# zkonduit/ezkl

Hardware: AMD Instinct MI355X
Metric: BN254 G1 MSM pts/s (2^20 points per GPU; NTT 2^22 elems/s in extra) (higher is better)
Workload: dtype u32x8 (254-bit modular integer, Montgomery); 1 GPU; configs[1]: standalone 2^20-point BN254 G1 MSM (uniform scalars, try-and-increment bases) + 2^22 scalar-field NTT per GPU; parallelism=points sharded across 1 rank(s); all_gather of 64-B partials + host fold

## Files before the change

ezkl_amd/csrc/field.hpp:

```cpp
#pragma once
#ifndef __HIPCC_RTC__
#include <stdint.h>
#include <hip/hip_runtime.h>
#else
typedef unsigned int uint32_t;
typedef unsigned long long uint64_t;
typedef unsigned long size_t;
#endif
#include "bn254_constants.h"

#define EZ_HD __host__ __device__ __forceinline__
#define EZ_D __device__ __forceinline__

namespace ezkl {

struct alignas(16) fe_t {
    uint32_t v[8];
};
#define EZKL_FE_DEFINED 1

struct FqP {
    static constexpr uint32_t MOD[8] = BN32_FQ_MOD_INIT;
    static constexpr uint32_t ONE[8] = BN32_FQ_R_INIT;
    static constexpr uint32_t R2[8] = BN32_FQ_R2_INIT;
// ... 134 lines not shown
    EZ_HD static fe_t sub_lazy(const fe_t& a, const fe_t& b) {
        fe_t d;
        uint32_t br = 0;
#pragma unroll
        for (int i = 0; i < 8; i++) d.v[i] = subb32(a.v[i], b.v[i], br);
        uint32_t c = 0;
        fe_t r;
#pragma unroll
        for (int i = 0; i < 8; i++) r.v[i] = addc32(d.v[i], mod2(i), c);
        return r;
    }
    __host__ __device__ __attribute__((noinline)) static u32x8 mul_lazy_call(u32x8 a, u32x8 b) {
        fe_t x, y;
#pragma unroll
        for (int i = 0; i < 8; i++) { x.v[i] = a[i]; y.v[i] = b[i]; }
#if defined(__HIP_DEVICE_COMPILE__)
        fe_t r;
        mont_mul_single<P>(x.v, y.v, r.v);
#else
        fe_t r = mul_portable(reduce_once(reduce_2p(x)), y);
#endif
        u32x8 o;
#pragma unroll
        for (int i = 0; i < 8; i++) o[i] = r.v[i];
        return o;
    }
    EZ_HD static fe_t mul_lazy(const fe_t& a, const fe_t& b) {
        u32x8 x, y;
#pragma unroll
        for (int i = 0; i < 8; i++) { x[i] = a.v[i]; y[i] = b.v[i]; }
        u32x8 o = mul_lazy_call(x, y);
        fe_t r;
#pragma unroll
        for (int i = 0; i < 8; i++) r.v[i] = o[i];
        return r;
    }
    EZ_HD static fe_t mul(const fe_t& a, const fe_t& b) {
        u32x8 x, y;
#pragma unroll
        for (int i = 0; i < 8; i++) { x[i] = a.v[i]; y[i] = b.v[i]; }
        u32x8 o = mul_call(x, y);
        fe_t r;
#pragma unroll
        for (int i = 0; i < 8; i++) r.v[i] = o[i];
        return r;
    }
    EZ_HD static fe_t mul_inl(const fe_t& a, const fe_t& b) {
#if defined(__HIP_DEVICE_COMPILE__)
        return mont_mul_asm<P>(a, b);
#else
        return mul_portable(a, b);
#endif
    }
    EZ_HD static fe_t mul_portable(const fe_t& a, const fe_t& b) {
        uint32_t t[8];
#pragma unroll
        for (int i = 0; i < 8; i++) t[i] = 0;
#pragma unroll
        for (int i = 0; i < 8; i++) {
            const uint32_t bi = b.v[i];
            uint64_t A = mad_wide(a.v[0], bi, t[0]);
            const uint32_t m = (uint32_t)A * P::INV;
            uint64_t C = mad_wide(m, P::MOD[0], (uint32_t)A);
#pragma unroll
            for (int j = 1; j < 8; j++) {
                A = mad_wide(a.v[j], bi, (uint64_t)t[j] + (A >> 32));
                C = mad_wide(m, P::MOD[j], (uint64_t)(uint32_t)A + (C >> 32));
                t[j - 1] = (uint32_t)C;
            }
            t[7] = (uint32_t)(A >> 32) + (uint32_t)(C >> 32);
        }
        fe_t r;
#pragma unroll
        for (int i = 0; i < 8; i++) r.v[i] = t[i];
        return reduce_once(r);
    }
    EZ_HD static fe_t sqr(const fe_t& a) { return mul(a, a); }

    EZ_HD static fe_t from_mont(const fe_t& a) {
        fe_t o = zero();
        o.v[0] = 1;
        return mul(a, o);
    }
    EZ_HD static fe_t to_mont(const fe_t& a) { return mul(a, r2()); }

    EZ_HD static fe_t pow(const fe_t& a, const uint32_t e[8]) {
        fe_t acc = one(), base = a;
        for (int i = 0; i < 256; i++) {
            if ((e[i >> 5] >> (i & 31)) & 1) acc = mul(acc, base);
            base = sqr(base);
        }
        return acc;
    }
    EZ_HD static fe_t pow_u64(const fe_t& a, uint64_t e) {
        fe_t acc = one(), base = a;
        while (e) {
            if (e & 1) acc = mul(acc, base);
            base = sqr(base);
            e >>= 1;
        }
        return acc;
    }
    EZ_HD static fe_t inv(const fe_t& a) {
        uint32_t e[8];
        uint64_t br = 2;
        for (int i = 0; i < 8; i++) {
            uint64_t t = (uint64_t)P::MOD[i] - br;
            e[i] = (uint32_t)t;
            br = (t >> 63) & 1;
        }
        return pow(a, e);
    }
    EZ_HD static fe_t from_u64(uint64_t x) {
        fe_t t = zero();
        t.v[0] = (uint32_t)x;
        t.v[1] = (uint32_t)(x >> 32);
        return to_mont(t);
    }
};

}
namespace ezkl {
#include "montmul_gen.hpp"
template <> __device__ __forceinline__ void mont_mul_single<FqP>(const uint32_t (&a)[8], const uint32_t (&b)[8], uint32_t (&r)[8]) { mont_mul_asm1_fq(a, b, r); }
template <> __device__ __forceinline__ void mont_mul_single<FrP>(const uint32_t (&a)[8], const uint32_t (&b)[8], uint32_t (&r)[8]) { mont_mul_asm1_fr(a, b, r); }
using Fr = Field<FrP>;
using Fq = Field<FqP>;

EZ_D fe_t ld_fe(const fe_t* p) {
    const uint4* q = reinterpret_cast<const uint4*>(p);
    uint4 lo = q[0], hi = q[1];
    fe_t r;
    r.v[0] = lo.x; r.v[1] = lo.y; r.v[2] = lo.z; r.v[3] = lo.w;
    r.v[4] = hi.x; r.v[5] = hi.y; r.v[6] = hi.z; r.v[7] = hi.w;
    return r;
}
EZ_D void st_fe(fe_t* p, const fe_t& a) {
    uint4* q = reinterpret_cast<uint4*>(p);
    q[0] = make_uint4(a.v[0], a.v[1], a.v[2], a.v[3]);
    q[1] = make_uint4(a.v[4], a.v[5], a.v[6], a.v[7]);
}

EZ_HD fe_t fr_const(const uint32_t (&c)[8]) {
    fe_t r;
#pragma unroll
    for (int i = 0; i < 8; i++) r.v[i] = c[i];
    return r;
}
struct FrConst {
    static constexpr uint32_t ROOT[8] = BN32_FR_ROOT_INIT;
    static constexpr uint32_t ZETA[8] = BN32_FR_ZETA_INIT;
    static constexpr uint32_t ZETA2[8] = BN32_FR_ZETA2_INIT;
    static constexpr uint32_t DELTA[8] = BN32_FR_DELTA_INIT;
};
struct FqConst {
    static constexpr uint32_t B3[8] = BN32_FQ_B3_INIT;
};

}
```

ezkl_amd/csrc/msm.hip:

```cpp
#include "common.hpp"
#include <deque>
#include <thread>
#include <chrono>
#include "curve.hpp"
#include "curve29.hpp"
#include "host64.hpp"
#include <string.h>

namespace ezkl {

static constexpr uint32_t MSM_MAX_PART_BITS = 12;
static constexpr uint32_t MSM_SPAN_HEAVY = 16;
static constexpr uint32_t MSM_PART_STAGE = 13312;
static constexpr uint32_t MSM_BINSORT_STAGE = 15360;
static constexpr uint32_t MSM_HEAVY_CHUNK = 256;
static constexpr uint32_t MSM_DIGIT_E = 8;
static constexpr uint32_t MSM_LMIN = 8;
static constexpr uint32_t MSM_MAX_BIG = 64;
static constexpr uint32_t MSM_BIG_BLOCKS = 64;
static constexpr uint32_t MSM_BIG_ROWS = 8;

__device__ __forceinline__ uint32_t msm_part_of(uint32_t bucket, uint32_t NP) { return bucket ? 1u + (bucket & (NP - 1u)) : 0u; }
__device__ __forceinline__ uint32_t msm_lane_len(const uint32_t* offsets, uint32_t nb, uint32_t nlanes, uint32_t lmin) {
    const uint32_t l = (uint32_t)(((uint64_t)offsets[nb] + nlanes - 1) / nlanes);
// ... 54 lines not shown
    return v;
}
static const int MSM_SLOTS = msm_slots_init();
struct MsmSlot {
    hipStream_t st = nullptr;
    uint8_t* scratch = nullptr;
    size_t scratch_bytes = 0;
    uint32_t* pinned = nullptr;
    void* pinned_dev = nullptr;
    size_t pinned_msms = 0;
    hipEvent_t done = nullptr;
    uint32_t bits = 0;
    uint32_t count = 0;
    void* out = nullptr;
    bool busy = false;
};
static constexpr int MSM_CALL_SLOTS = 4;
struct MsmState {
    std::map<const Bases*, MsmTable> tables;
    hipStream_t table_stream = nullptr;
    MsmSlot slots[MSM_MAX_SLOTS];
    MsmSlot call_slots[MSM_CALL_SLOTS];
    bool call_claimed[MSM_CALL_SLOTS] = {false, false, false, false};
    bool call_finishing[MSM_CALL_SLOTS] = {false, false, false, false};
    std::thread::id call_owner[MSM_CALL_SLOTS];
    hipEvent_t call_order_ev = nullptr;
    hipStream_t copy_st = nullptr;
    fe_t* tail_pinned = nullptr;
    size_t tail_pinned_elems = 0;
    MsmUpload* open_upload = nullptr;
    MsmBatch* open_batch = nullptr;
    bool attrs_set = false;
    int acc_blocks_per_cu = 0;
};
static MsmState& msm_state() {
    Ctx* c = ctx();
    if (!c->msm_state) c->msm_state = new MsmState();
    return *static_cast<MsmState*>(c->msm_state);
}


static WinPlan pick_plan(size_t n) {
    WinPlan best{0, 0, 0};
    double best_cost = 0;
    for (uint32_t W = 10; W <= 127; W++) {
        WinPlan p{W, 254 / W, 254 % W};
        if (p.cmax() > 23) continue;
        const double cost = (double)n * W + 4.0 * (double)((size_t)1 << (p.cmax() - 1));
        if (!best.W || cost < best_cost) { best = p; best_cost = cost; }
    }
    return best;
}

__global__ __launch_bounds__(256) void msm_precompute_kernel(const g1a_t* prev, g1a_t* next, size_t n, uint32_t c) {
    size_t i = (size_t)blockIdx.x * blockDim.x + threadIdx.x;
    if (i >= n) return;
    g1a_t p = ld_g1a(prev + i);
    g1x_t a = g1x_from_affine(p);
    for (uint32_t k = 0; k < c; k++) a = g1x_double(a);
    st_g1a(next + i, g1x_to_affine(a));
}

__global__ __launch_bounds__(256) void msm_table_to_r261_kernel(g1a_t* tab, size_t count) {
    size_t i = (size_t)blockIdx.x * blockDim.x + threadIdx.x;
    if (i >= count) return;
    fe_t k;
#pragma unroll
    for (int q = 0; q < 8; q++) k.v[q] = Fq29C::R261_32[q];
    g1a_t p = ld_g1a(tab + i);
    if (g1a_is_id(p)) return;
    p.x = Fq::mul(p.x, k);
    p.y = Fq::mul(p.y, k);
    st_g1a(tab + i, p);
}

__device__ __forceinline__ bool gt_half_r(const fe_t& s) {
    uint32_t d[8], c = 0, br = 0;
#pragma unroll
    for (int i = 0; i < 8; i++) d[i] = addc32(s.v[i], s.v[i], c);
#pragma unroll
    for (int i = 0; i < 8; i++) (void)subb32(d[i], FrP::MOD[i], br);
    return c != 0 || br == 0;
}
__device__ __forceinline__ fe_t msm_canon(const fe_t* scalars, size_t i, uint32_t& neg) {
    fe_t s = Fr::from_mont(ld_fe(scalars + i));
    neg = 0;
    if (gt_half_r(s)) {
        uint32_t br = 0;
#pragma unroll
        for (int k = 0; k < 8; k++) s.v[k] = subb32(FrP::MOD[k], s.v[k], br);
        neg = 1;
    }
    return s;
}
__device__ __forceinline__ uint32_t msm_take_bits(fe_t& s, uint32_t c) {
    const uint32_t d = s.v[0] & ((1u << c) - 1u);
#pragma unroll
    for (int k = 0; k < 7; k++) s.v[k] = __builtin_amdgcn_alignbit(s.v[k + 1], s.v[k], c);
    s.v[7] >>= c;
    return d;
}
template <class F>
__device__ __forceinline__ void msm_foreach_digit(fe_t s, uint32_t neg, const WinPlan& wp, F&& f) {
    uint32_t carry = 0;
    for (uint32_t w = 0; w < wp.W; w++) {
        const uint32_t c = wp.width(w), half = 1u << (c - 1);
        uint32_t raw = msm_take_bits(s, c) + carry;
        if (raw > half) {
            carry = 1;
            if (raw != (1u << c)) f(w, (1u << c) - raw - 1u, neg ^ 1u);
        } else {
            carry = 0;
            if (raw) f(w, raw - 1u, neg);
        }
    }
}

__device__ __forceinline__ bool msm_digit_step(fe_t& s, uint32_t neg, uint32_t c, uint32_t& carry, uint32_t& bucket, uint32_t& sign) {
    const uint32_t half = 1u << (c - 1);
    const uint32_t raw = msm_take_bits(s, c) + carry;
    if (raw > half) {
        carry = 1;
        bucket = (1u << c) - raw - 1u;
        sign = neg ^ 1u;
        return raw != (1u << c);
    }
    carry = 0;
    bucket = raw - 1u;
    sign = neg;
    return raw != 0;
}

__device__ __forceinline__ uint32_t msm_block_scan(uint32_t v, uint32_t* wsum, uint32_t& total) {
    const uint32_t lane = threadIdx.x & 63u, wave = threadIdx.x >> 6, nw = blockDim.x >> 6;
    uint32_t x = v;
#pragma unroll
    for (uint32_t d = 1; d < 64; d <<= 1) {
        const uint32_t y = __shfl_up(x, d, 64);
        if (lane >= d) x += y;
    }
    if (lane == 63) wsum[wave] = x;
    __syncthreads();
    if (wave == 0) {
        uint32_t s = lane < nw ? wsum[lane] : 0u;
#pragma unroll
        for (uint32_t d = 1; d < 16; d <<= 1) {
            const uint32_t y = __shfl_up(s, d, 64);
            if (lane >= d) s += y;
        }
        if (lane < nw) wsum[lane] = s;
    }
    __syncthreads();
    total = wsum[nw - 1];
    const uint32_t r = x + (wave ? wsum[wave - 1] : 0u);
    __syncthreads();
    return r;
}

__global__ __launch_bounds__(256) void msm_hist_kernel(MsmCols cols, size_t n, size_t per_block, WinPlan wp,
                                                       uint32_t LB, uint32_t NP, uint32_t* wg_hist, uint32_t* wg_cnt,
                                                       uint32_t* zero_base, uint32_t zero_words, size_t bstride) {
    BOFF(); BSH(wg_hist); BSH(wg_cnt);
    const fe_t* scalars = msm_col(cols);
    if (zero_base) {
        BSH(zero_base);
        for (uint32_t i = blockIdx.x * 256 + threadIdx.x; i < zero_words; i += gridDim.x * 256) zero_base[i] = 0;
    }
    __shared__ uint32_t lh[(1u << MSM_MAX_PART_BITS) + 1];
    const uint32_t NQ = NP + 1;
    for (uint32_t p = threadIdx.x; p < NQ; p += 256) lh[p] = 0;
    __syncthreads();
    size_t lo = (size_t)blockIdx.x * per_block, hi = lo + per_block < n ? lo + per_block : n;
    for (size_t i0 = lo + threadIdx.x; i0 < hi; i0 += 4 * 256) {
        fe_t s[4];
        uint32_t neg[4], carry[4] = {0, 0, 0, 0};
#pragma unroll
        for (int q = 0; q < 4; q++) {
            const size_t i = i0 + (size_t)q * 256;
            if (i < hi) s[q] = msm_canon(scalars, i, neg[q]);
            else { s[q] = Fr::zero(); neg[q] = 0; }
        }
        for (uint32_t w = 0; w < wp.W; w++) {
            const uint32_t c = wp.width(w);
#pragma unroll
            for (int q = 0; q < 4; q++) {
                uint32_t bucket, sign;
                if (msm_digit_step(s[q], neg[q], c, carry[q], bucket, sign)) atomicAdd(&lh[msm_part_of(bucket, NP)], 1u);
            }
        }
    }
    __syncthreads();
    for (uint32_t p = threadIdx.x; p < NQ; p += 256) {
        wg_hist[(size_t)blockIdx.x * NQ + p] = lh[p];
        wg_cnt[(size_t)blockIdx.x * NQ + p] = lh[p];
    }
}
__global__ __launch_bounds__(1024) void msm_hist_scan_kernel(uint32_t* wg_hist, uint32_t G, uint32_t NP, uint32_t* part_count, size_t bstride) {
    BOFF(); BSH(wg_hist); BSH(part_count);
    __shared__ uint32_t sums[32][33];
    const uint32_t c = threadIdx.x & 31, j = threadIdx.x >> 5;
    const uint32_t p = blockIdx.x * 32 + c;
    const uint32_t chunk = (G + 31) / 32, g0 = j * chunk, g1 = g0 + chunk < G ? g0 + chunk : G;
    uint32_t s = 0;
    if (p < NP)
        for (uint32_t g = g0; g < g1; g++) s += wg_hist[(size_t)g * NP + p];
    sums[j][c] = s;
    __syncthreads();
    if (j == 0) {
        uint32_t run = 0;
        for (uint32_t q = 0; q < 32; q++) {
            uint32_t v = sums[q][c];
            sums[q][c] = run;
            run += v;
        }
        if (p < NP) part_count[p] = run;
    }
    __syncthreads();
    if (p < NP) {
        uint32_t run = sums[j][c];
        for (uint32_t g = g0; g < g1; g++) {
            uint32_t v = wg_hist[(size_t)g * NP + p];
            wg_hist[(size_t)g * NP + p] = run;
            run += v;
        }
    }
}
__device__ __forceinline__ void msm_part_scan_body(const uint32_t* part_count, uint32_t NQ, uint32_t* part_base, uint32_t* big_flag,
                                                   uint32_t* big_list, uint32_t* big_count, uint32_t* sh) {
    const uint32_t t = threadIdx.x;
    constexpr uint32_t PER = 5;
    uint32_t v[PER], sum = 0;
#pragma unroll
    for (uint32_t q = 0; q < PER; q++) {
        const uint32_t i = PER * t + q;
        v[q] = i < NQ ? part_count[i] : 0;
        sum += v[q];
    }
    uint32_t total;
    uint32_t run = msm_block_scan(sum, sh, total) - sum;
#pragma unroll
    for (uint32_t q = 0; q < PER; q++) {
        const uint32_t i = PER * t + q;
        if (i < NQ) part_base[i] = run;
        run += v[q];
    }
    if (t == 1023) part_base[NQ] = total;
#pragma unroll
    for (uint32_t q = 0; q < PER; q++) {
        const uint32_t i = PER * t + q;
        if (i == 0 || i >= NQ) continue;
        uint32_t slot = 0;
        if (v[q] > MSM_BINSORT_STAGE) {
            slot = atomicAdd(big_count, 1u);
            if (slot < MSM_MAX_BIG) big_list[slot] = i - 1;
            slot = slot < MSM_MAX_BIG ? slot + 1 : 0;
        }
        big_flag[i - 1] = slot;
    }
}
__global__ __launch_bounds__(1024) void msm_part_scan_kernel(const uint32_t* part_count, uint32_t NQ, uint32_t* part_base, uint32_t* big_flag,
                                                             uint32_t* big_list, uint32_t* big_count, size_t bstride) {
    BOFF(); BSH(part_count); BSH(part_base); BSH(big_flag); BSH(big_list); BSH(big_count);
    __shared__ uint32_t sh[1024];
    msm_part_scan_body(part_count, NQ, part_base, big_flag, big_list, big_count, sh);
}
__global__ __launch_bounds__(1024) void msm_partition_kernel(MsmCols cols, size_t n, size_t per_block, WinPlan wp,
                                                             uint32_t LB, uint32_t NP, size_t base_offset, size_t tab_stride,
                                                             const uint32_t* part_base, const uint32_t* wg_hist, const uint32_t* wg_cnt, uint2* entries,
                                                             uint32_t* vals, size_t bstride) {
    BOFF(); BSH(part_base); BSH(wg_hist); BSH(wg_cnt); BSH(entries); BSH(vals);
    const fe_t* scalars = msm_col(cols);
    extern __shared__ uint32_t plds[];
    __shared__ uint32_t tsum[1024];
    const uint32_t NQ = NP + 1;
    uint32_t* start = plds;
    uint32_t* cursor = plds + (NQ + 1);
    uint32_t* gbase = plds + 2 * (NQ + 1);
    uint2* stage = reinterpret_cast<uint2*>(plds + 3 * (NQ + 1));
    const uint32_t t = threadIdx.x, T = blockDim.x;
    const uint32_t K = (NQ + T - 1) / T;
    uint32_t loc = 0;
    for (uint32_t q = 0; q < K; q++) {
        const uint32_t p = t * K + q;
        if (p < NQ) loc += wg_cnt[(size_t)blockIdx.x * NQ + p];
    }
    uint32_t total;
    uint32_t run = msm_block_scan(loc, tsum, total) - loc;
    for (uint32_t q = 0; q < K; q++) {
        const uint32_t p = t * K + q;
        if (p < NQ) {
            start[p] = run;
            cursor[p] = run;
            gbase[p] = part_base[p] + wg_hist[(size_t)blockIdx.x * NQ + p];
            run += wg_cnt[(size_t)blockIdx.x * NQ + p];
        }
    }
    __syncthreads();
    const size_t lo = (size_t)blockIdx.x * per_block, hi = lo + per_block < n ? lo + per_block : n;
    const size_t i = lo + t;
    if (i < hi) {
        uint32_t neg;
        fe_t s = msm_canon(scalars, i, neg);
        msm_foreach_digit(s, neg, wp, [&](uint32_t w, uint32_t bucket, uint32_t sign) {
            const uint32_t r = atomicAdd(&cursor[msm_part_of(bucket, NP)], 1u);
            stage[r] = make_uint2((uint32_t)(w * tab_stride + base_offset + i) | (sign << 31), bucket);
        });
    }
    __syncthreads();
    const uint32_t PB = 31 - __clz(NP);
    for (uint32_t idx = t; idx < total; idx += T) {
        const uint2 e = stage[idx];
        const uint32_t p = msm_part_of(e.y, NP);
        const uint32_t slot = gbase[p] + (idx - start[p]);
        if (p) entries[slot] = make_uint2(e.x, e.y >> PB);
        else vals[slot] = e.x;
    }
}
__device__ __forceinline__ uint32_t msm_wave_rank(uint32_t* cnt, uint32_t key) {
    const uint64_t active = __ballot(1);
    const uint32_t first = __builtin_amdgcn_readfirstlane(key);
    if (__ballot(key == first) == active) {
        const uint32_t rank = (uint32_t)__popcll(active & ((1ull << (threadIdx.x & 63u)) - 1ull));
        uint32_t base = 0;
        if (rank == 0) base = atomicAdd(&cnt[first], (uint32_t)__popcll(active));
        return (uint32_t)__builtin_amdgcn_readfirstlane(base) + rank;
    }
    return atomicAdd(&cnt[key], 1u);
}
__device__ __forceinline__ void msm_bins_scan(uint32_t* cnt, uint32_t* tsum, uint32_t nbins, uint32_t p, uint32_t beg, const uint32_t* part_base,
                                              bool emit, uint32_t* offsets, g1x29_t* buckets) {
    const uint32_t t = threadIdx.x;
    uint32_t loc[4], s = 0;
#pragma unroll
    for (int q = 0; q < 4; q++) {
        uint32_t j = t * 4 + q;
        loc[q] = j < nbins ? cnt[j] : 0;
        s += loc[q];
    }
    uint32_t total;
    uint32_t run = msm_block_scan(s, tsum, total) - s;
#pragma unroll
    for (int q = 0; q < 4; q++) {
        uint32_t j = t * 4 + q;
        if (j < nbins) {
            cnt[j] = run;
            if (emit) {
                const bool b0 = (p == 0 && j == 0);
                offsets[(size_t)p * nbins + j] = b0 ? part_base[0] : beg + run;
                if (b0 ? part_base[1] == part_base[0] : loc[q] == 0) st_f29(&buckets[(size_t)p * nbins + j].zz, Fq29::zero());
            }
        }
        run += loc[q];
    }
    __syncthreads();
}
__device__ __forceinline__ void msm_bigsort_count_body(const uint2* entries, const uint32_t* part_base, uint32_t LB, const uint32_t* big_list,
                                                       const uint32_t* big_count, uint32_t* bin_total, uint32_t* block_off, uint32_t* cnt, uint32_t bx,
                                                       uint32_t by, uint32_t rows);
__global__ __launch_bounds__(512) void msm_binsort_kernel(const uint2* entries, const uint32_t* part_base, uint32_t LB, uint32_t NP,
                                                          const uint32_t* big_flag, uint32_t* offsets, uint32_t* vals, g1x29_t* buckets,
                                                          const uint32_t* big_list, const uint32_t* big_count, uint32_t* bin_total, uint32_t* block_off,
                                                          size_t bstride) {
    BOFF(); BSH(entries); BSH(part_base); BSH(big_flag); BSH(offsets); BSH(vals); BSH(buckets);
    __shared__ uint32_t cnt[2048];
    __shared__ uint32_t tsum[512];
    extern __shared__ uint32_t stage[];
    if (blockIdx.x >= NP) {
        BSH(big_list); BSH(big_count); BSH(bin_total); BSH(block_off);
        const uint32_t w = blockIdx.x - NP;
        msm_bigsort_count_body(entries, part_base, LB, big_list, big_count, bin_total, block_off, cnt, w % MSM_BIG_BLOCKS, w / MSM_BIG_BLOCKS, MSM_BIG_ROWS);
        return;
    }
    const uint32_t p = blockIdx.x, t = threadIdx.x, nbins = 1u << LB;
    const uint32_t beg = part_base[p + 1], end = part_base[p + 2];
    if (p == NP - 1 && t == 0) offsets[(size_t)NP * nbins] = end;
    if (big_flag[p]) return;
    const bool staged = (end - beg) <= MSM_BINSORT_STAGE;
    for (uint32_t j = t; j < nbins; j += 512) cnt[j] = 0;
    __syncthreads();
    if (staged) {
        constexpr int PER = MSM_BINSORT_STAGE / 512;
        uint2 v[PER];
#pragma unroll
        for (int q = 0; q < PER; q++) {
            const uint32_t e = beg + t + (uint32_t)q * 512u;
            v[q] = e < end ? entries[e] : make_uint2(0u, 0xffffffffu);
        }
#pragma unroll
        for (int q = 0; q < PER; q++)
            if (v[q].y != 0xffffffffu) atomicAdd(&cnt[v[q].y], 1u);
        __syncthreads();
        msm_bins_scan(cnt, tsum, nbins, p, beg, part_base, true, offsets, buckets);
#pragma unroll
        for (int q = 0; q < PER; q++)
            if (v[q].y != 0xffffffffu) stage[atomicAdd(&cnt[v[q].y], 1u)] = v[q].x;
        __syncthreads();
        for (uint32_t i = t; i < end - beg; i += 512) vals[beg + i] = stage[i];
    } else {
// ... 382 lines not shown
static size_t msm_group_size(const MsmTable* T, size_t n, bool small_scalars, size_t batch = 0) {
    if (const char* e = getenv("EZKL_MSM_GROUP")) {
        const int v = atoi(e);
        if (v >= 1 && v <= (int)MSM_MAX_GROUP) return (size_t)v;
    }
    (void)T; (void)n; (void)batch;
    if (small_scalars) {
        static const int small = [] { const char* e = getenv("EZKL_MSM_GROUP_SMALL"); const int v = e ? atoi(e) : 0; return v >= 1 && v <= (int)MSM_MAX_GROUP ? v : 6; }();
        return (size_t)small;
    }
    static const int big = [] { const char* e = getenv("EZKL_MSM_GROUP_BIG"); const int v = e ? atoi(e) : 0; return v >= 1 && v <= (int)MSM_MAX_GROUP ? v : 4; }();
    return (size_t)big;
}
static int msm_enqueue(Ctx* c, MsmSlot& sl, hipStream_t st, MsmTable* T, size_t base_offset, const fe_t* const* cols, size_t count, size_t n, bool timed) {
    int rc = EZKL_OK;
    if (count < 1 || count > MSM_MAX_GROUP) return EZKL_ERR_INVALID;
    const unsigned Z = (unsigned)count;
    const WinPlan wp = T->wp;
    const uint32_t W = wp.W, bits = wp.cmax() - 1;
    const uint32_t nb = 1u << bits;
    const size_t npairs = n * W;
    uint32_t PB = bits < 10 ? bits : 10;
    while (PB < bits && PB < MSM_MAX_PART_BITS && (npairs >> PB) > (size_t)MSM_BINSORT_STAGE * 9 / 10) PB++;
    const uint32_t LB = bits - PB, NP = 1u << PB;
    int& acc_blocks_per_cu = msm_state().acc_blocks_per_cu;
    if (!acc_blocks_per_cu) {
        EZ_HIP(hipFuncSetAttribute((const void*)msm_binsort_kernel, hipFuncAttributeMaxDynamicSharedMemorySize, 96 * 1024));
        EZ_HIP(hipFuncSetAttribute((const void*)msm_partition_kernel, hipFuncAttributeMaxDynamicSharedMemorySize, 144 * 1024));
        EZ_HIP(hipOccupancyMaxActiveBlocksPerMultiprocessor(&acc_blocks_per_cu, msm_accumulate_kernel, 256, 0));
        if (acc_blocks_per_cu < 1) acc_blocks_per_cu = 1;
    }
    const size_t resident = (size_t)acc_blocks_per_cu * 256 * c->num_cus;
    const size_t load = npairs >> bits, per_lane = load * 9 / 10 > 40 ? load * 9 / 10 : 40;
    size_t rounds = npairs / (resident * per_lane);
    if (rounds < 1) rounds = 1;
    uint32_t L = (uint32_t)((npairs + resident * rounds - 1) / (resident * rounds));
    if (L < 8) L = 8;
    if (const char* e = getenv("EZKL_MSM_L")) {
        const int v = atoi(e);
        if (v > 0 && v < (1 << 20)) L = (uint32_t)v;
    }
    const uint32_t nlanes = cdiv(npairs, L);
    static const uint32_t lmin = [] { const char* e = getenv("EZKL_MSM_LMIN"); const int v = e ? atoi(e) : 0; return (uint32_t)(v >= 1 && v <= 4096 ? v : (int)MSM_LMIN); }();
    constexpr uint32_t coop = 7;
    static const uint32_t span_heavy = [] { const char* e = getenv("EZKL_MSM_SPAN"); const int v = e ? atoi(e) : 0; return (uint32_t)(v >= 1 && v <= 4096 ? v : (int)MSM_SPAN_HEAVY); }();
    ReduceGeom rg;
    memset(&rg, 0, sizeof rg);
    if (LB > 0) {
        rg.wA = LB; rg.wsA = PB;
        rg.wB = (PB + 1) / 2; rg.wsB = 0;
        rg.wC = PB - rg.wB; rg.wsC = rg.wB;
    } else {
        rg.wA = (bits + 2) / 3; rg.wsA = 0;
        rg.wB = (bits - rg.wA + 1) / 2; rg.wsB = rg.wA;
        rg.wC = bits - rg.wA - rg.wB; rg.wsC = rg.wA + rg.wB;
    }
    {
        const uint32_t rows = 1u << (rg.wB + rg.wC), cols = 1u << rg.wA;
        uint32_t E = MSM_DIGIT_E;
        if (const char* e = getenv("EZKL_MSM_E")) {
            const int v = atoi(e);
            if (v > 0 && v <= 1024 && (v & (v - 1)) == 0) E = (uint32_t)v;
        }
        rg.EA = rows < E ? rows : E; rg.GA = rows / rg.EA;
        rg.ET = cols < E ? cols : E; rg.GT = cols / rg.ET;
    }
    const uint32_t nA = 1u << rg.wA, nT = 1u << (rg.wB + rg.wC);
    const uint32_t n_partA = nA * rg.GA, n_partT = nT * rg.GT;
    const uint32_t nplanes = 1 + bits;
    size_t per_block = MSM_PART_STAGE / W / 64 * 64;
    {
        const size_t lds_words = (144u << 10) / 4, fixed = 3 * ((size_t)NP + 2);
        const size_t fit = lds_words > fixed ? (lds_words - fixed) / (2 * (size_t)W) / 64 * 64 : 64;
        if (per_block > fit) per_block = fit;
    }
    if (per_block > 1024) per_block = 1024;
    if (per_block < 64) per_block = 64;
    const unsigned sgrid = cdiv(n, per_block);
    auto al = [](size_t x) { return (x + 255) & ~(size_t)255; };
    size_t off = 0;
    auto carve = [&](size_t bytes) { size_t o = off; off += al(bytes); return o; };
    size_t o_ent = carve(npairs * 8), o_vals = carve(npairs * 4), o_offs = carve(((size_t)nb + 1) * 4);
    const uint32_t NQ = NP + 1;
    size_t o_pcnt = carve((NQ + 1) * 4), o_pbase = carve((NQ + 1) * 4), o_wgh = carve((size_t)sgrid * NQ * 4), o_wgc = carve((size_t)sgrid * NQ * 4);
    size_t o_heavy = carve((size_t)nb * 4), o_chunks = carve(((size_t)nlanes + 1) * 4);
    const size_t nbins = (size_t)1 << LB;
    size_t o_hcnt = carve(256), o_btot = carve(MSM_MAX_BIG * nbins * 4), o_planes = carve((size_t)nplanes * sizeof(g1x29_t));
    const size_t zero_bytes = off - o_hcnt;
    size_t o_bflag = carve((size_t)NP * 4), o_blist = carve(MSM_MAX_BIG * 4),
           o_boff = carve((size_t)MSM_MAX_BIG * MSM_BIG_BLOCKS * nbins * 4);
    size_t o_lfirst = carve((size_t)nlanes * 4);
    size_t o_bkt = carve((size_t)nb * sizeof(g1x29_t));
    size_t o_head = carve((size_t)nlanes * sizeof(g1x29_t)), o_tail = carve((size_t)nlanes * sizeof(g1x29_t));
    size_t o_partA = carve((size_t)n_partA * sizeof(g1x29_t)), o_partT = carve((size_t)n_partT * sizeof(g1x29_t));
    size_t o_SA = carve((size_t)nA * sizeof(g1x29_t)), o_T = carve((size_t)nT * sizeof(g1x29_t));
    const size_t bstride = count > 1 ? off : 0;
    rc = slot_prepare(sl, off * count, count);
    if (rc) return rc;
    uint8_t* S = sl.scratch;
    MsmCols kcols;
    for (size_t j = 0; j < MSM_MAX_GROUP; j++) kcols.col[j] = cols[j < count ? j : 0];
    uint2* entries = (uint2*)(S + o_ent);
    uint32_t* vals = (uint32_t*)(S + o_vals);
    uint32_t* offs = (uint32_t*)(S + o_offs);
    uint32_t *pcnt = (uint32_t*)(S + o_pcnt), *pbase = (uint32_t*)(S + o_pbase), *wghist = (uint32_t*)(S + o_wgh), *wgcnt = (uint32_t*)(S + o_wgc);
    uint32_t *heavy = (uint32_t*)(S + o_heavy), *hcnt = (uint32_t*)(S + o_hcnt), *chunks = (uint32_t*)(S + o_chunks);
    uint32_t* lfirst = (uint32_t*)(S + o_lfirst);
    uint32_t *bflag = (uint32_t*)(S + o_bflag), *blist = (uint32_t*)(S + o_blist), *btot = (uint32_t*)(S + o_btot), *boff = (uint32_t*)(S + o_boff);
    uint32_t* bcnt = hcnt + 2;
    g1x29_t *bkt = (g1x29_t*)(S + o_bkt), *head = (g1x29_t*)(S + o_head), *tail = (g1x29_t*)(S + o_tail);
    g1x29_t *partA = (g1x29_t*)(S + o_partA), *partT = (g1x29_t*)(S + o_partT), *SA = (g1x29_t*)(S + o_SA), *TT = (g1x29_t*)(S + o_T);
    g1x29_t* planes = (g1x29_t*)(S + o_planes);

    hipEvent_t m0 = nullptr, m1 = nullptr, a0 = nullptr, a1 = nullptr;
    bool timed_chain = timed;
    if (timed) {
        const char* tm = getenv("EZKL_HIP_TIMING");
        if (tm && !strcmp(tm, "none")) timed = timed_chain = false;
        else if (tm && !strcmp(tm, "kernel")) timed_chain = false;
    }
    if (timed) {
        if (timed_chain && (rc = ev_pair(c, "msm", &m0, &m1))) return rc;
        if ((rc = ev_pair(c, "msm_accumulate", &a0, &a1))) return rc;
        if (timed_chain) EZ_HIP(hipEventRecord(m0, st));
    }
    hipLaunchKernelGGL(msm_hist_kernel, dim3(sgrid, 1, Z), dim3(256), 0, st, kcols, n, per_block, wp, LB, NP, wghist, wgcnt, hcnt,
                       (uint32_t)(zero_bytes / 4), bstride);
    hipLaunchKernelGGL(msm_hist_scan_kernel, dim3(cdiv(NQ, 32), 1, Z), dim3(1024), 0, st, wghist, sgrid, NQ, pcnt, bstride);
    hipLaunchKernelGGL(msm_part_scan_kernel, dim3(1, 1, Z), dim3(1024), 0, st, pcnt, NQ, pbase, bflag, blist, bcnt, bstride);
    hipLaunchKernelGGL(msm_partition_kernel, dim3(sgrid, 1, Z), dim3((unsigned)per_block), (3 * ((size_t)NQ + 1) + 2 * per_block * W) * 4, st, kcols, n, per_block, wp,
                       LB, NP, base_offset, T->n, pbase, wghist, wgcnt, entries, vals, bstride);
    hipLaunchKernelGGL(msm_binsort_kernel, dim3(NP + MSM_BIG_BLOCKS * MSM_BIG_ROWS, 1, Z), dim3(512), MSM_BINSORT_STAGE * 4, st, entries, pbase, LB, NP, bflag, offs,
                       vals, bkt, blist, bcnt, btot, boff, bstride);
    hipLaunchKernelGGL(msm_bigsort_scatter_kernel, dim3(MSM_BIG_BLOCKS, MSM_BIG_ROWS, Z), dim3(512), 0, st, entries, pbase, LB, blist, bcnt, btot, boff, offs,
                       vals, bkt, bstride);
    if (timed) EZ_HIP(hipEventRecord(a0, st));
    hipLaunchKernelGGL(msm_accumulate_kernel, dim3(cdiv(nlanes, 256), 1, Z), dim3(256), 0, st, T->tab, offs, vals, nb, nlanes, bkt, head, tail,
                       lfirst, lmin, bstride);
    if (timed) EZ_HIP(hipEventRecord(a1, st));
    if (nlanes > 1)
    {
        hipLaunchKernelGGL(msm_fixup_boundary_tree_kernel, dim3(cdiv(nlanes - 1, 256), 1, Z), dim3(256), 0, st, offs, nb, nlanes, lfirst, head, tail, bkt,
                           heavy, hcnt, chunks, lmin, span_heavy, bstride);
    }
    {
        size_t max_heavy = nlanes / span_heavy + 1;
        const size_t heavy_wgs = (max_heavy + 3) / 4;
        unsigned hb = (unsigned)(heavy_wgs < (size_t)c->num_cus * 4 ? heavy_wgs : (size_t)c->num_cus * 4);
        size_t max_chunks = nlanes / MSM_HEAVY_CHUNK + max_heavy;
        const size_t chunk_wgs = (max_chunks + 3) / 4;
        unsigned cb = (unsigned)(chunk_wgs < (size_t)c->num_cus * 4 ? chunk_wgs : (size_t)c->num_cus * 4);
        hipLaunchKernelGGL(msm_fixup_heavy1_kernel, dim3(cb, 1, Z), dim3(256), 0, st, offs, nb, nlanes, lfirst, head, tail, bkt, chunks, hcnt, lmin, coop & 4u, bstride);
        hipLaunchKernelGGL(msm_fixup_heavy2_kernel, dim3(hb, 1, Z), dim3(256), 0, st, offs, nb, nlanes, head, tail, heavy, hcnt, bkt, lmin, coop & 4u, bstride);
    }
    {
        const uint32_t th = n_partA > n_partT ? n_partA : n_partT;
        hipLaunchKernelGGL(msm_reduce1_kernel, dim3(cdiv(th, 256), 2, Z), dim3(256), 0, st, bkt, rg, partA, partT, bstride);
        auto pow2_le = [](uint32_t x) { uint32_t p = 1; while (p * 2 <= x) p *= 2; return p; };
        uint32_t lanesA = pow2_le(rg.GA < 64 ? rg.GA : 64), lanesT = pow2_le(rg.GT < 64 ? rg.GT : 64);
        auto waves = [&](uint32_t nout, uint32_t lanes) { return cdiv(nout, 64 / lanes); };
        while (waves(nA, lanesA) + waves(nT, lanesT) > (unsigned)c->num_cus * 4 && (lanesA > 1 || lanesT > 1)) {
            if (lanesT > 1 && waves(nT, lanesT) >= waves(nA, lanesA)) lanesT >>= 1; else if (lanesA > 1) lanesA >>= 1; else lanesT >>= 1;
        }
        const uint32_t blocksA = waves(nA, lanesA);
        hipLaunchKernelGGL(msm_reduce2_kernel, dim3(blocksA + waves(nT, lanesT), 1, Z), dim3(64), 0, st, partA, partT, rg, SA, TT, lanesA, lanesT, blocksA, coop & 1u, bstride);
        hipLaunchKernelGGL(msm_planes_kernel, dim3(nplanes, 1, Z), dim3(256), 0, st, SA, TT, rg, planes, (g1x29_t*)sl.pinned_dev,
                           coop & 10u, bstride);
    }
    EZ_HIP(hipGetLastError());
    if (getenv("EZKL_MSM_DEBUG")) {
        uint32_t hc = 0;
        EZ_HIP(hipMemcpyAsync(&hc, hcnt, 4, hipMemcpyDeviceToHost, st));
        EZ_HIP(hipStreamSynchronize(st));
        fprintf(stderr, "[msm] n=%zu W=%u bits=%u L=%u nlanes=%u heavy=%u\n", n, W, bits, L, nlanes, hc);
    }
    if (timed_chain) EZ_HIP(hipEventRecord(m1, st));
    EZ_HIP(hipEventRecord(sl.done, st));
    sl.bits = bits;
    sl.count = (uint32_t)count;
    sl.busy = true;
    return EZKL_OK;
}
static int msm_run_groups(Ctx* c, MsmTable* T, size_t base_offset, const fe_t* const* cols, size_t batch, size_t n, void* out_host,
                          const hipEvent_t* wait_ev, bool small_scalars) {
    const size_t G = msm_group_size(T, n, small_scalars, batch);
    static const bool dbg = getenv("EZKL_MSM_DEBUG") != nullptr;
    if (dbg) fprintf(stderr, "[ezkl_hip] msm batch: %zu columns of %zu points, %s scalars, groups of %zu\n", batch, n, small_scalars ? "witness-shaped" : "general", G);
    int rc = EZKL_OK;
    size_t gi = 0;
    for (size_t j0 = 0; j0 < batch && !rc; gi++) {
        size_t cnt = batch - j0 < G ? batch - j0 : G;
        if (wait_ev && j0 > 0) {
            const size_t left = batch - j0;
            cnt = left <= 2 ? 1 : std::min(G, (left + 1) / 2);
        }
        MsmSlot& sl = g_slots[gi % MSM_SLOTS];
        if (sl.busy) rc = msm_finish(sl);
        if (!rc) rc = slot_prepare(sl, 0);
        for (size_t j = 0; wait_ev && j < cnt && !rc; j++)
            if (hipStreamWaitEvent(sl.st, wait_ev[j0 + j], 0) != hipSuccess) rc = EZKL_ERR_HIP;
        if (!rc) {
            sl.out = (uint8_t*)out_host + 64 * j0;
            rc = msm_enqueue(c, sl, sl.st, T, base_offset, cols + j0, cnt, n, false);
        }
        j0 += cnt;
    }
    for (size_t k = 0; k < (size_t)MSM_SLOTS; k++) {
        MsmSlot& sl = g_slots[(gi + k) % MSM_SLOTS];
        if (!sl.busy) continue;
        if (!rc) rc = msm_finish(sl);
        else { (void)hipStreamSynchronize(sl.st); sl.busy = false; }
    }
    return rc;
}
// ... 464 lines not shown
```

Baseline: 811.4 million pts/s.

## Rework MSM scalar recoding, histogram scan and persistent partition kernel

Replaces from_mont (a full Montgomery multiply by one) with a dedicated REDC, and replaces the per-window shifting of all eight limbs with a streaming 64-bit buffer recoder that extracts signed digits for several scalars at once. The duplicated per-workgroup count array is dropped: the partition kernel now recovers per-tile counts by differencing adjacent exclusive-scan rows, with the partition totals serving as the last row. The histogram scan is rebuilt as a narrow-column wave-shuffle scan with XCD-aware strip mapping. The partition kernel is made persistent, with a grid capped at the CU count, and prefetches the next tile's scalars and histogram rows. The aim is to cut scalar-decoding ALU work and memory traffic in the sort front-end, at the cost of more complex indexing and less parallelism in the partition launch.

After: 822.1 million pts/s (median of 6 runs). 1.3% higher.

```diff
diff --git a/ezkl_amd/csrc/field.hpp b/ezkl_amd/csrc/field.hpp
--- a/ezkl_amd/csrc/field.hpp
+++ b/ezkl_amd/csrc/field.hpp
@@ -240,6 +240,26 @@
         o.v[0] = 1;
         return mul(a, o);
     }
+    EZ_HD static fe_t redc(const fe_t& a) {
+        uint32_t t[8];
+#pragma unroll
+        for (int i = 0; i < 8; i++) t[i] = a.v[i];
+#pragma unroll
+        for (int i = 0; i < 8; i++) {
+            const uint32_t m = t[0] * P::INV;
+            uint64_t pr[8];
+#pragma unroll
+            for (int j = 0; j < 8; j++) pr[j] = mad_wide(m, P::MOD[j], t[j]);
+            uint32_t c = 0;
+#pragma unroll
+            for (int j = 0; j < 7; j++) t[j] = addc32((uint32_t)pr[j + 1], (uint32_t)(pr[j] >> 32), c);
+            t[7] = (uint32_t)(pr[7] >> 32) + c;
+        }
+        fe_t r;
+#pragma unroll
+        for (int i = 0; i < 8; i++) r.v[i] = t[i];
+        return reduce_once(r);
+    }
     EZ_HD static fe_t to_mont(const fe_t& a) { return mul(a, r2()); }
 
     EZ_HD static fe_t pow(const fe_t& a, const uint32_t e[8]) {
diff --git a/ezkl_amd/csrc/msm.hip b/ezkl_amd/csrc/msm.hip
--- a/ezkl_amd/csrc/msm.hip
+++ b/ezkl_amd/csrc/msm.hip
@@ -160,8 +160,8 @@
     for (int i = 0; i < 8; i++) (void)subb32(d[i], FrP::MOD[i], br);
     return c != 0 || br == 0;
 }
-__device__ __forceinline__ fe_t msm_canon(const fe_t* scalars, size_t i, uint32_t& neg) {
-    fe_t s = Fr::from_mont(ld_fe(scalars + i));
+__device__ __forceinline__ fe_t msm_canon(const fe_t& mont, uint32_t& neg) {
+    fe_t s = Fr::redc(mont);
     neg = 0;
     if (gt_half_r(s)) {
         uint32_t br = 0;
@@ -171,42 +171,34 @@
     }
     return s;
 }
-__device__ __forceinline__ uint32_t msm_take_bits(fe_t& s, uint32_t c) {
-    const uint32_t d = s.v[0] & ((1u << c) - 1u);
-#pragma unroll
-    for (int k = 0; k < 7; k++) s.v[k] = __builtin_amdgcn_alignbit(s.v[k + 1], s.v[k], c);
-    s.v[7] >>= c;
-    return d;
-}
-template <class F>
-__device__ __forceinline__ void msm_foreach_digit(fe_t s, uint32_t neg, const WinPlan& wp, F&& f) {
-    uint32_t carry = 0;
-    for (uint32_t w = 0; w < wp.W; w++) {
-        const uint32_t c = wp.width(w), half = 1u << (c - 1);
-        uint32_t raw = msm_take_bits(s, c) + carry;
-        if (raw > half) {
-            carry = 1;
-            if (raw != (1u << c)) f(w, (1u << c) - raw - 1u, neg ^ 1u);
-        } else {
-            carry = 0;
-            if (raw) f(w, raw - 1u, neg);
-        }
-    }
-}
-
-__device__ __forceinline__ bool msm_digit_step(fe_t& s, uint32_t neg, uint32_t c, uint32_t& carry, uint32_t& bucket, uint32_t& sign) {
-    const uint32_t half = 1u << (c - 1);
-    const uint32_t raw = msm_take_bits(s, c) + carry;
-    if (raw > half) {
-        carry = 1;
-        bucket = (1u << c) - raw - 1u;
-        sign = neg ^ 1u;
-        return raw != (1u << c);
-    }
-    carry = 0;
-    bucket = raw - 1u;
-    sign = neg;
-    return raw != 0;
+template <int Q, class F>
+__device__ __forceinline__ void msm_recode(const fe_t (&s)[Q], const uint32_t (&neg)[Q], const WinPlan& wp, F&& f) {
+    uint64_t buf[Q];
+    uint32_t carry[Q];
+#pragma unroll
+    for (int q = 0; q < Q; q++) { buf[q] = 0; carry[q] = 0; }
+    uint32_t have = 0, w = 0, c = wp.width(0);
+#pragma unroll
+    for (int k = 0; k < 8; k++) {
+#pragma unroll
+        for (int q = 0; q < Q; q++) buf[q] |= (uint64_t)s[q].v[k] << have;
+        have += 32;
+        while (have >= c && w < wp.W) {
+            const uint32_t full = 1u << c, half = full >> 1;
+#pragma unroll
+            for (int q = 0; q < Q; q++) {
+                const uint32_t raw = ((uint32_t)buf[q] & (full - 1u)) + carry[q];
+                buf[q] >>= c;
+                const uint32_t minus = raw > half ? 1u : 0u;
+                const uint32_t mag = minus ? full - raw : raw;
+                carry[q] = minus;
+                if (mag) f(q, w, mag - 1u, neg[q] ^ minus);
+            }
+            have -= c;
+            w++;
+            c = wp.width(w);
+        }
+    }
 }
 
 __device__ __forceinline__ uint32_t msm_block_scan(uint32_t v, uint32_t* wsum, uint32_t& total) {
@@ -236,9 +228,9 @@
 }
 
 __global__ __launch_bounds__(256) void msm_hist_kernel(MsmCols cols, size_t n, size_t per_block, WinPlan wp,
-                                                       uint32_t LB, uint32_t NP, uint32_t* wg_hist, uint32_t* wg_cnt,
+                                                       uint32_t LB, uint32_t NP, uint32_t* wg_hist,
                                                        uint32_t* zero_base, uint32_t zero_words, size_t bstride) {
-    BOFF(); BSH(wg_hist); BSH(wg_cnt);
+    BOFF(); BSH(wg_hist);
     const fe_t* scalars = msm_col(cols);
     if (zero_base) {
         BSH(zero_base);
@@ -251,56 +243,77 @@
     size_t lo = (size_t)blockIdx.x * per_block, hi = lo + per_block < n ? lo + per_block : n;
     for (size_t i0 = lo + threadIdx.x; i0 < hi; i0 += 4 * 256) {
         fe_t s[4];
-        uint32_t neg[4], carry[4] = {0, 0, 0, 0};
+        uint32_t neg[4];
 #pragma unroll
         for (int q = 0; q < 4; q++) {
             const size_t i = i0 + (size_t)q * 256;
-            if (i < hi) s[q] = msm_canon(scalars, i, neg[q]);
-            else { s[q] = Fr::zero(); neg[q] = 0; }
-        }
-        for (uint32_t w = 0; w < wp.W; w++) {
-            const uint32_t c = wp.width(w);
-#pragma unroll
-            for (int q = 0; q < 4; q++) {
-                uint32_t bucket, sign;
-                if (msm_digit_step(s[q], neg[q], c, carry[q], bucket, sign)) atomicAdd(&lh[msm_part_of(bucket, NP)], 1u);
-            }
-        }
+            s[q] = i < hi ? ld_fe(scalars + i) : Fr::zero();
+        }
+#pragma unroll
+        for (int q = 0; q < 4; q++) s[q] = msm_canon(s[q], neg[q]);
+        msm_recode<4>(s, neg, wp, [&](int, uint32_t, uint32_t bucket, uint32_t) { atomicAdd(&lh[msm_part_of(bucket, NP)], 1u); });
     }
     __syncthreads();
-    for (uint32_t p = threadIdx.x; p < NQ; p += 256) {
-        wg_hist[(size_t)blockIdx.x * NQ + p] = lh[p];
-        wg_cnt[(size_t)blockIdx.x * NQ + p] = lh[p];
-    }
-}
+    for (uint32_t p = threadIdx.x; p < NQ; p += 256) wg_hist[(size_t)blockIdx.x * NQ + p] = lh[p];
+}
+static constexpr uint32_t MSM_SCAN_COLS = 4;
 __global__ __launch_bounds__(1024) void msm_hist_scan_kernel(uint32_t* wg_hist, uint32_t G, uint32_t NP, uint32_t* part_count, size_t bstride) {
     BOFF(); BSH(wg_hist); BSH(part_count);
-    __shared__ uint32_t sums[32][33];
-    const uint32_t c = threadIdx.x & 31, j = threadIdx.x >> 5;
-    const uint32_t p = blockIdx.x * 32 + c;
-    const uint32_t chunk = (G + 31) / 32, g0 = j * chunk, g1 = g0 + chunk < G ? g0 + chunk : G;
-    uint32_t s = 0;
-    if (p < NP)
-        for (uint32_t g = g0; g < g1; g++) s += wg_hist[(size_t)g * NP + p];
-    sums[j][c] = s;
+    __shared__ uint32_t wsum[64];
+    const uint32_t t = threadIdx.x, lane = t & 63u, wave = t >> 6;
+    const uint32_t c = t & (MSM_SCAN_COLS - 1u), j = t / MSM_SCAN_COLS;
+    const uint32_t nstrips = gridDim.x, sq = nstrips / 8, sr = nstrips % 8, xcd = blockIdx.x % 8;
+    const uint32_t strip = (xcd < sr ? xcd * (sq + 1) : sr * (sq + 1) + (xcd - sr) * sq) + blockIdx.x / 8;
+    const uint32_t p = strip * MSM_SCAN_COLS + c;
+    const uint32_t chunk = (G + 255) / 256, g0 = j * chunk, g1 = p < NP ? (g0 + chunk < G ? g0 + chunk : G) : 0;
+    uint32_t v[8], sum = 0;
+#pragma unroll
+    for (uint32_t q = 0; q < 8; q++) v[q] = g0 + q < g1 ? wg_hist[(size_t)(g0 + q) * NP + p] : 0u;
+#pragma unroll
+    for (uint32_t q = 0; q < 8; q++) sum += v[q];
+    for (uint32_t gb = g0 + 8; gb < g1; gb += 8) {
+        uint32_t u[8];
+#pragma unroll
+        for (uint32_t q = 0; q < 8; q++) u[q] = gb + q < g1 ? wg_hist[(size_t)(gb + q) * NP + p] : 0u;
+#pragma unroll
+        for (uint32_t q = 0; q < 8; q++) sum += u[q];
+    }
+    uint32_t x = sum;
+#pragma unroll
+    for (uint32_t d = MSM_SCAN_COLS; d < 64; d <<= 1) {
+        const uint32_t y = __shfl_up(x, d, 64);
+        if (lane >= d) x += y;
+    }
+    if (lane >= 64 - MSM_SCAN_COLS) wsum[wave * MSM_SCAN_COLS + c] = x;
     __syncthreads();
-    if (j == 0) {
-        uint32_t run = 0;
-        for (uint32_t q = 0; q < 32; q++) {
-            uint32_t v = sums[q][c];
-            sums[q][c] = run;
-            run += v;
-        }
-        if (p < NP) part_count[p] = run;
+    if (wave == 0) {
+        uint32_t s = wsum[lane];
+#pragma unroll
+        for (uint32_t d = MSM_SCAN_COLS; d < 64; d <<= 1) {
+            const uint32_t y = __shfl_up(s, d, 64);
+            if (lane >= d) s += y;
+        }
+        wsum[lane] = s;
     }
     __syncthreads();
-    if (p < NP) {
-        uint32_t run = sums[j][c];
-        for (uint32_t g = g0; g < g1; g++) {
-            uint32_t v = wg_hist[(size_t)g * NP + p];
-            wg_hist[(size_t)g * NP + p] = run;
-            run += v;
-        }
+    uint32_t run = x - sum + (wave ? wsum[(wave - 1) * MSM_SCAN_COLS + c] : 0u);
+    if (j == 0 && p < NP) part_count[p] = wsum[15 * MSM_SCAN_COLS + c];
+#pragma unroll
+    for (uint32_t q = 0; q < 8; q++)
+        if (g0 + q < g1) {
+            wg_hist[(size_t)(g0 + q) * NP + p] = run;
+            run += v[q];
+        }
+    for (uint32_t gb = g0 + 8; gb < g1; gb += 8) {
+        uint32_t u[8];
+#pragma unroll
+        for (uint32_t q = 0; q < 8; q++) u[q] = gb + q < g1 ? wg_hist[(size_t)(gb + q) * NP + p] : 0u;
+#pragma unroll
+        for (uint32_t q = 0; q < 8; q++)
+            if (gb + q < g1) {
+                wg_hist[(size_t)(gb + q) * NP + p] = run;
+                run += u[q];
+            }
     }
 }
 __device__ __forceinline__ void msm_part_scan_body(const uint32_t* part_count, uint32_t NQ, uint32_t* part_base, uint32_t* big_flag,
@@ -342,11 +355,12 @@
     __shared__ uint32_t sh[1024];
     msm_part_scan_body(part_count, NQ, part_base, big_flag, big_list, big_count, sh);
 }
-__global__ __launch_bounds__(1024) void msm_partition_kernel(MsmCols cols, size_t n, size_t per_block, WinPlan wp,
+static constexpr uint32_t MSM_PART_PF = 2;
+__global__ __launch_bounds__(1024) void msm_partition_kernel(MsmCols cols, size_t n, size_t per_block, uint32_t G, WinPlan wp,
                                                              uint32_t LB, uint32_t NP, size_t base_offset, size_t tab_stride,
-                                                             const uint32_t* part_base, const uint32_t* wg_hist, const uint32_t* wg_cnt, uint2* entries,
+                                                             const uint32_t* part_base, const uint32_t* wg_hist, const uint32_t* part_count, uint2* entries,
                                                              uint32_t* vals, size_t bstride) {
-    BOFF(); BSH(part_base); BSH(wg_hist); BSH(wg_cnt); BSH(entries); BSH(vals);
+    BOFF(); BSH(part_base); BSH(wg_hist); BSH(part_count); BSH(entries); BSH(vals);
     const fe_t* scalars = msm_col(cols);
     extern __shared__ uint32_t plds[];
     __shared__ uint32_t tsum[1024];
@@ -357,41 +371,73 @@
     uint2* stage = reinterpret_cast<uint2*>(plds + 3 * (NQ + 1));
     const uint32_t t = threadIdx.x, T = blockDim.x;
     const uint32_t K = (NQ + T - 1) / T;
-    uint32_t loc = 0;
-    for (uint32_t q = 0; q < K; q++) {
-        const uint32_t p = t * K + q;
-        if (p < NQ) loc += wg_cnt[(size_t)blockIdx.x * NQ + p];
-    }
-    uint32_t total;
-    uint32_t run = msm_block_scan(loc, tsum, total) - loc;
-    for (uint32_t q = 0; q < K; q++) {
-        const uint32_t p = t * K + q;
-        if (p < NQ) {
-            start[p] = run;
-            cursor[p] = run;
-            gbase[p] = part_base[p] + wg_hist[(size_t)blockIdx.x * NQ + p];
-            run += wg_cnt[(size_t)blockIdx.x * NQ + p];
-        }
-    }
-    __syncthreads();
-    const size_t lo = (size_t)blockIdx.x * per_block, hi = lo + per_block < n ? lo + per_block : n;
-    const size_t i = lo + t;
-    if (i < hi) {
-        uint32_t neg;
-        fe_t s = msm_canon(scalars, i, neg);
-        msm_foreach_digit(s, neg, wp, [&](uint32_t w, uint32_t bucket, uint32_t sign) {
-            const uint32_t r = atomicAdd(&cursor[msm_part_of(bucket, NP)], 1u);
-            stage[r] = make_uint2((uint32_t)(w * tab_stride + base_offset + i) | (sign << 31), bucket);
-        });
-    }
-    __syncthreads();
     const uint32_t PB = 31 - __clz(NP);
-    for (uint32_t idx = t; idx < total; idx += T) {
-        const uint2 e = stage[idx];
-        const uint32_t p = msm_part_of(e.y, NP);
-        const uint32_t slot = gbase[p] + (idx - start[p]);
-        if (p) entries[slot] = make_uint2(e.x, e.y >> PB);
-        else vals[slot] = e.x;
+    auto row = [&](uint32_t tile, uint32_t p) { return wg_hist[(size_t)tile * NQ + p]; };
+    auto row_next = [&](uint32_t tile, uint32_t p) { return tile + 1 < G ? wg_hist[(size_t)(tile + 1) * NQ + p] : part_count[p]; };
+    fe_t sm[1];
+    uint32_t h0[MSM_PART_PF], h1[MSM_PART_PF];
+    auto fetch = [&](uint32_t tile) {
+        const size_t lo = (size_t)tile * per_block, hi = lo + per_block < n ? lo + per_block : n;
+        sm[0] = lo + t < hi ? ld_fe(scalars + lo + t) : Fr::zero();
+#pragma unroll
+        for (uint32_t q = 0; q < MSM_PART_PF; q++) {
+            const uint32_t p = t * K + q;
+            const bool in = q < K && p < NQ;
+            h0[q] = in ? row(tile, p) : 0u;
+            h1[q] = in ? row_next(tile, p) : 0u;
+        }
+    };
+    if (blockIdx.x < G) fetch(blockIdx.x);
+    for (uint32_t tile = blockIdx.x; tile < G; tile += gridDim.x) {
+        uint32_t loc = 0;
+#pragma unroll
+        for (uint32_t q = 0; q < MSM_PART_PF; q++) loc += h1[q] - h0[q];
+        for (uint32_t q = MSM_PART_PF; q < K; q++) {
+            const uint32_t p = t * K + q;
+            if (p < NQ) loc += row_next(tile, p) - row(tile, p);
+        }
+        uint32_t total;
+        uint32_t run = msm_block_scan(loc, tsum, total) - loc;
+#pragma unroll
+        for (uint32_t q = 0; q < MSM_PART_PF; q++) {
+            const uint32_t p = t * K + q;
+            if (q < K && p < NQ) {
+                start[p] = run;
+                cursor[p] = run;
+                gbase[p] = part_base[p] + h0[q];
+                run += h1[q] - h0[q];
+            }
+        }
+        for (uint32_t q = MSM_PART_PF; q < K; q++) {
+            const uint32_t p = t * K + q;
+            if (p < NQ) {
+                const uint32_t r0 = row(tile, p);
+                start[p] = run;
+                cursor[p] = run;
+                gbase[p] = part_base[p] + r0;
+                run += row_next(tile, p) - r0;
+            }
+        }
+        __syncthreads();
+        const size_t lo = (size_t)tile * per_block, hi = lo + per_block < n ? lo + per_block : n;
+        const size_t i = lo + t;
+        if (i < hi) {
+            uint32_t neg[1];
+            sm[0] = msm_canon(sm[0], neg[0]);
+            msm_recode<1>(sm, neg, wp, [&](int, uint32_t w, uint32_t bucket, uint32_t sign) {
+                const uint32_t r = atomicAdd(&cursor[msm_part_of(bucket, NP)], 1u);
+                stage[r] = make_uint2((uint32_t)(w * tab_stride + base_offset + i) | (sign << 31), bucket);
+            });
+        }
+        __syncthreads();
+        if (tile + gridDim.x < G) fetch(tile + gridDim.x);
+        for (uint32_t idx = t; idx < total; idx += T) {
+            const uint2 e = stage[idx];
+            const uint32_t p = msm_part_of(e.y, NP);
+            const uint32_t slot = gbase[p] + (idx - start[p]);
+            if (p) entries[slot] = make_uint2(e.x, e.y >> PB);
+            else vals[slot] = e.x;
+        }
     }
 }
 __device__ __forceinline__ uint32_t msm_wave_rank(uint32_t* cnt, uint32_t key) {
@@ -940,7 +986,7 @@
     auto carve = [&](size_t bytes) { size_t o = off; off += al(bytes); return o; };
     size_t o_ent = carve(npairs * 8), o_vals = carve(npairs * 4), o_offs = carve(((size_t)nb + 1) * 4);
     const uint32_t NQ = NP + 1;
-    size_t o_pcnt = carve((NQ + 1) * 4), o_pbase = carve((NQ + 1) * 4), o_wgh = carve((size_t)sgrid * NQ * 4), o_wgc = carve((size_t)sgrid * NQ * 4);
+    size_t o_pcnt = carve((NQ + 1) * 4), o_pbase = carve((NQ + 1) * 4), o_wgh = carve((size_t)sgrid * NQ * 4);
     size_t o_heavy = carve((size_t)nb * 4), o_chunks = carve(((size_t)nlanes + 1) * 4);
     const size_t nbins = (size_t)1 << LB;
     size_t o_hcnt = carve(256), o_btot = carve(MSM_MAX_BIG * nbins * 4), o_planes = carve((size_t)nplanes * sizeof(g1x29_t));
@@ -961,7 +1007,7 @@
     uint2* entries = (uint2*)(S + o_ent);
     uint32_t* vals = (uint32_t*)(S + o_vals);
     uint32_t* offs = (uint32_t*)(S + o_offs);
-    uint32_t *pcnt = (uint32_t*)(S + o_pcnt), *pbase = (uint32_t*)(S + o_pbase), *wghist = (uint32_t*)(S + o_wgh), *wgcnt = (uint32_t*)(S + o_wgc);
+    uint32_t *pcnt = (uint32_t*)(S + o_pcnt), *pbase = (uint32_t*)(S + o_pbase), *wghist = (uint32_t*)(S + o_wgh);
     uint32_t *heavy = (uint32_t*)(S + o_heavy), *hcnt = (uint32_t*)(S + o_hcnt), *chunks = (uint32_t*)(S + o_chunks);
     uint32_t* lfirst = (uint32_t*)(S + o_lfirst);
     uint32_t *bflag = (uint32_t*)(S + o_bflag), *blist = (uint32_t*)(S + o_blist), *btot = (uint32_t*)(S + o_btot), *boff = (uint32_t*)(S + o_boff);
@@ -982,12 +1028,13 @@
         if ((rc = ev_pair(c, "msm_accumulate", &a0, &a1))) return rc;
         if (timed_chain) EZ_HIP(hipEventRecord(m0, st));
     }
-    hipLaunchKernelGGL(msm_hist_kernel, dim3(sgrid, 1, Z), dim3(256), 0, st, kcols, n, per_block, wp, LB, NP, wghist, wgcnt, hcnt,
+    hipLaunchKernelGGL(msm_hist_kernel, dim3(sgrid, 1, Z), dim3(256), 0, st, kcols, n, per_block, wp, LB, NP, wghist, hcnt,
                        (uint32_t)(zero_bytes / 4), bstride);
-    hipLaunchKernelGGL(msm_hist_scan_kernel, dim3(cdiv(NQ, 32), 1, Z), dim3(1024), 0, st, wghist, sgrid, NQ, pcnt, bstride);
+    hipLaunchKernelGGL(msm_hist_scan_kernel, dim3(cdiv(NQ, MSM_SCAN_COLS), 1, Z), dim3(1024), 0, st, wghist, sgrid, NQ, pcnt, bstride);
     hipLaunchKernelGGL(msm_part_scan_kernel, dim3(1, 1, Z), dim3(1024), 0, st, pcnt, NQ, pbase, bflag, blist, bcnt, bstride);
-    hipLaunchKernelGGL(msm_partition_kernel, dim3(sgrid, 1, Z), dim3((unsigned)per_block), (3 * ((size_t)NQ + 1) + 2 * per_block * W) * 4, st, kcols, n, per_block, wp,
-                       LB, NP, base_offset, T->n, pbase, wghist, wgcnt, entries, vals, bstride);
+    const unsigned pgrid = sgrid < (unsigned)c->num_cus ? sgrid : (unsigned)c->num_cus;
+    hipLaunchKernelGGL(msm_partition_kernel, dim3(pgrid, 1, Z), dim3((unsigned)per_block), (3 * ((size_t)NQ + 1) + 2 * per_block * W) * 4, st, kcols, n, per_block,
+                       (uint32_t)sgrid, wp, LB, NP, base_offset, T->n, pbase, wghist, pcnt, entries, vals, bstride);
     hipLaunchKernelGGL(msm_binsort_kernel, dim3(NP + MSM_BIG_BLOCKS * MSM_BIG_ROWS, 1, Z), dim3(512), MSM_BINSORT_STAGE * 4, st, entries, pbase, LB, NP, bflag, offs,
                        vals, bkt, blist, bcnt, btot, boff, bstride);
     hipLaunchKernelGGL(msm_bigsort_scatter_kernel, dim3(MSM_BIG_BLOCKS, MSM_BIG_ROWS, Z), dim3(512), 0, st, entries, pbase, LB, blist, bcnt, btot, boff, offs,
```
